# Quantum-Chemistry-Group-BNU/PyNQS

Hardware: AMD Instinct MI355X
Metric: local energies/sec (whole node) (higher is better)
Workload: dtype f64

## Files before the change

### pynqs_amd/csrc/kernels_reduce_rowout.hip

```cpp
#include "reduce_list.h"

namespace pynqs {

template <int LEN, typename T>
#ifndef PYNQS_ROWOUT_WAVES
#define PYNQS_ROWOUT_WAVES 6
#endif
__global__ __launch_bounds__(kBlock) __attribute__((amdgpu_waves_per_eu(PYNQS_ROWOUT_WAVES, 8)))
void reduce_onepass_list_rowout_kernel(const uint64_t *__restrict__ bra, SDParams p, PlanLayout pl, uint32_t nchunks, uint32_t chunk_len, uint32_t max_tiles,
                                       const T *__restrict__ plan, T eps, uint32_t nsample, uint64_t seed, uint32_t P, OnepassOut<T> o) {
  reduce_onepass_list_body<LEN, T, true, false, false, false, true>(bra, p, pl, nchunks, chunk_len, max_tiles, plan, eps, nsample, seed, P, o);
}

template <int LEN, typename T, bool GTILE>
__global__ __launch_bounds__(kBlock) void reduce_onepass_list_flush_row32_kernel(const uint64_t *__restrict__ bra, SDParams p, PlanLayout pl, uint32_t nchunks,
                                                                                uint32_t chunk_len, uint32_t max_tiles, const T *__restrict__ plan, T eps,
                                                                                uint32_t nsample, uint64_t seed, uint32_t P, OnepassOut<T> o) {
  reduce_onepass_list_body<LEN, T, true, false, true, GTILE, false, true>(bra, p, pl, nchunks, chunk_len, max_tiles, plan, eps, nsample, seed, P, o);
}

int launch_reduce_flush_row32(const uint64_t *bra, int64_t nbatch, const SDParams &p, const PlanLayout &pl, uint32_t chunk_len, uint32_t max_tiles,
                              const void *plan, int dtype, double eps_eff, int eps_sample, uint64_t seed, uint32_t P, size_t lds,
                              const pynqs_reduce_io *io, uint32_t fixed, bool gtile, hipStream_t st) {
  if (!io->row_f32) return set_error(PYNQS_EINVAL, "io->row_f32 missing");
  const int len = (p.sorb - 1) / 64 + 1;
#define PYNQS_R32_LAUNCH(TT)                                                                                                             \
  do {                                                                                                                                   \
    auto kfn = gtile ? reduce_onepass_list_flush_row32_kernel<LEN, TT, true> : reduce_onepass_list_flush_row32_kernel<LEN, TT, false>;   \
    if (lds > 64 * 1024 && hipFuncSetAttribute(reinterpret_cast<const void *>(kfn), hipFuncAttributeMaxDynamicSharedMemorySize, (int)lds) != hipSuccess) \
      return check_launch("hipFuncSetAttribute");                                                                                       \
    hipLaunchKernelGGL(kfn, dim3((uint32_t)nbatch), dim3(kBlock), lds, st, bra, p, pl, 1u, chunk_len, max_tiles, (const TT *)plan, (TT)eps_eff, \
                       (uint32_t)eps_sample, seed, P, make_out<TT>(io, len, fixed, gtile ? max_tiles : 0u));                            \
  } while (0)
  DISPATCH_LEN(len, {
    if (dtype == PYNQS_F64) PYNQS_R32_LAUNCH(double); else PYNQS_R32_LAUNCH(float);
  });
#undef PYNQS_R32_LAUNCH
  return check_launch("reduce_onepass (semi-stochastic, flushing, float32 row copy)");
}

bool reduce_draw_supported(const SDParams &p, int eps_sample) {
  return eps_sample > 0 && (uint32_t)eps_sample <= kDrawMaxDraws && p.nsd + 1 <= kDrawMaxCols;
}

int launch_reduce_rowout(const uint64_t *bra, int64_t nbatch, const SDParams &p, const PlanLayout &pl, uint32_t chunk_len, uint32_t max_tiles,
                         const void *plan, int dtype, double eps_eff, int eps_sample, uint64_t seed, uint32_t P, size_t lds,
                         const pynqs_reduce_io *io, uint32_t fixed, hipStream_t st) {
  if (!io->row_f32) return set_error(PYNQS_EINVAL, "io->row_f32 missing");
  const int len = (p.sorb - 1) / 64 + 1;
#define PYNQS_RO_LAUNCH(TT)                                                                                                              \
  do {                                                                                                                                   \
    auto kfn = reduce_onepass_list_rowout_kernel<LEN, TT>;                                                                               \
    if (lds > 64 * 1024 && hipFuncSetAttribute(reinterpret_cast<const void *>(kfn), hipFuncAttributeMaxDynamicSharedMemorySize, (int)lds) != hipSuccess) \
      return check_launch("hipFuncSetAttribute");                                                                                       \
    hipLaunchKernelGGL(kfn, dim3((uint32_t)nbatch), dim3(kBlock), lds, st, bra, p, pl, 1u, chunk_len, max_tiles, (const TT *)plan, (TT)eps_eff, \
                       (uint32_t)eps_sample, seed, P, make_out<TT>(io, len, fixed, 0u));                                                 \
  } while (0)
  DISPATCH_LEN(len, {
    if (dtype == PYNQS_F64) PYNQS_RO_LAUNCH(double); else PYNQS_RO_LAUNCH(float);
  });
#undef PYNQS_RO_LAUNCH
  return check_launch("reduce_onepass (semi-stochastic, sorted draws)");
}

}

#ifdef PYNQS_OP_STAMPS
extern "C" int pynqs_debug_stamps(unsigned long long *out) {
  return (int)hipMemcpyFromSymbol(out, HIP_SYMBOL(pynqs::g_stamps), sizeof(unsigned long long) * 8192 * 16);
}
#endif
```

### pynqs_amd/csrc/reduce_draw.h

```cpp
#pragma once
#include "reduce_common.h"

namespace pynqs {

constexpr int kDrawSeg = 16;
constexpr uint32_t kDrawMaxCols = 2u * kBlock * kDrawSeg, kDrawMaxDraws = 16383;
constexpr uint32_t kNoRec = 0xffffffffu;

__host__ __device__ inline size_t draw_lds_bytes(uint32_t nsample) {
  auto al = [](size_t b) { return (b + 15) & ~(size_t)15; };
  (void)nsample;
  return al((size_t)(2 * kBlock + 1) * 8) + (size_t)kBlock * 8;
}
__host__ __device__ inline size_t draw_row_stride(uint32_t ncomb) { return ((size_t)ncomb + kDrawSeg - 1) & ~(size_t)(kDrawSeg - 1); }

template <typename T, int K>
__device__ __forceinline__ void probe_k_oneword(const OnepassOut<T> &o, const uint64_t (&ket)[K][1], const bool (&act)[K], int32_t (&lk)[K],
                                                bool (&won)[K], int32_t (&rowhint)[K], uint32_t *full_flag) {
  uint32_t s[K];
  bool open[K];
  const bool full = *full_flag != 0u;
#pragma unroll
  for (int k = 0; k < K; ++k) {
    won[k] = false; rowhint[k] = -1;
    open[k] = act[k] && !full && !(o.debug & 1u);
    if (act[k]) lk[k] = -1;
    s[k] = (uint32_t)(hash_of<1>(ket[k]) >> 17) & o.dedup_mask;
  }
  for (uint32_t probes = 0;; ++probes) {
    unsigned long long cur[K];
    int32_t rw[K];
    if constexpr (K == 4) {
      typedef uint32_t u4 __attribute__((ext_vector_type(4)));
      u4 x0, x1, x2, x3;
      const uint64_t *a0 = o.dedup + (open[0] ? (size_t)s[0] * 2 : 0), *a1 = o.dedup + (open[1] ? (size_t)s[1] * 2 : 0),
                     *a2 = o.dedup + (open[2] ? (size_t)s[2] * 2 : 0), *a3 = o.dedup + (open[3] ? (size_t)s[3] * 2 : 0);
      asm volatile("global_load_dwordx4 %0, %4, off sc1\n\t"
                   "global_load_dwordx4 %1, %5, off sc1\n\t"
                   "global_load_dwordx4 %2, %6, off sc1\n\t"
                   "global_load_dwordx4 %3, %7, off sc1\n\t"
                   "s_waitcnt vmcnt(0)"
                   : "=&v"(x0), "=&v"(x1), "=&v"(x2), "=&v"(x3)
                   : "v"(a0), "v"(a1), "v"(a2), "v"(a3)
                   : "memory");
      cur[0] = ((unsigned long long)x0[1] << 32) | x0[0]; rw[0] = (int32_t)x0[2];
      cur[1] = ((unsigned long long)x1[1] << 32) | x1[0]; rw[1] = (int32_t)x1[2];
      cur[2] = ((unsigned long long)x2[1] << 32) | x2[0]; rw[2] = (int32_t)x2[2];
      cur[3] = ((unsigned long long)x3[1] << 32) | x3[0]; rw[3] = (int32_t)x3[2];
    } else {
#pragma unroll
      for (int k = 0; k < K; ++k) {
        cur[k] = 0ull; rw[k] = -1;
        if (open[k]) {
          unsigned long long *kp = reinterpret_cast<unsigned long long *>(o.dedup + (size_t)s[k] * 2);
          cur[k] = __hip_atomic_load(kp, __ATOMIC_RELAXED, __HIP_MEMORY_SCOPE_AGENT);
          rw[k] = __hip_atomic_load(reinterpret_cast<int32_t *>(kp + 1), __ATOMIC_RELAXED, __HIP_MEMORY_SCOPE_AGENT);
        }
      }
    }
#pragma unroll
    for (int k = 0; k < K; ++k) {
      if (open[k] && cur[k] == ~0ull && (o.debug & 2048u)) { open[k] = false; continue; }
      if (open[k] && cur[k] == ~0ull) {
        unsigned long long *kp = reinterpret_cast<unsigned long long *>(o.dedup + (size_t)s[k] * 2);
        cur[k] = atomicCAS(kp, ~0ull, (unsigned long long)ket[k][0]);
        if (cur[k] == ~0ull) { won[k] = true; lk[k] = (int32_t)s[k]; open[k] = false; }
        else rw[k] = -1;
      }
    }
    bool any = false;
#pragma unroll
    for (int k = 0; k < K; ++k) {
      if (open[k]) {
        if (cur[k] == ket[k][0]) { lk[k] = (int32_t)s[k]; rowhint[k] = rw[k]; open[k] = false; }
        else { s[k] = (s[k] + 1) & o.dedup_mask; any = true; }
      }
    }
    if (!any) break;
    if (probes + 1 >= kProbeLimit) {
      atomicOr(reinterpret_cast<unsigned int *>(o.counters + 1), 2u);
      *full_flag = 1u;
      break;
    }
  }
}

template <typename V>
__device__ __forceinline__ V draw_block_scan(V v, V *s_part, V *total) {
  const int lane = threadIdx.x & 63, wave = threadIdx.x >> 6;
  V incl = v;
#pragma unroll
  for (int d = 1; d < 64; d <<= 1) {
    const V ov = __shfl_up(incl, d);
    if (lane >= d) incl += ov;
  }
  __syncthreads();
  if (lane == 63) s_part[wave] = incl;
  __syncthreads();
  V before = V(0), tot = V(0);
#pragma unroll
  for (int w = 0; w < kBlock / 64; ++w) {
    if (w < wave) before += s_part[w];
    tot += s_part[w];
  }
  *total = tot;
  return before + incl;
}

template <int LEN, typename T>
__device__ __forceinline__ void rowout_draws(unsigned char *lds, uint32_t *rec, const uint32_t *kcol, uint32_t nkept, int64_t seg_base, const SDParams &p,
                                             const LdsLayout &L, const Walker<LEN> &wk, const float *__restrict__ w, uint32_t nsample, uint64_t seed,
                                             uint64_t walker, double Srow, const OnepassOut<T> &o, uint32_t *bw_cnt, int32_t *bw_base, uint32_t *s_full,
                                             double *s_part, uint32_t *s_parti) {
  constexpr int NT = kBlock, K = 4, SEG = kDrawSeg;
  typedef float f4 __attribute__((ext_vector_type(4)));
  const int tid = threadIdx.x;
  const uint32_t ncomb = p.nsd + 1;
  const uint32_t nseg = (ncomb + SEG - 1) / SEG, nbw = (ncomb + 31) / 32;
  const int64_t sbase = (int64_t)walker * nsample;
  auto al = [](size_t b) { return (b + 15) & ~(size_t)15; };
  double *pfx = reinterpret_cast<double *>(lds);
  uint32_t *bitmap = reinterpret_cast<uint32_t *>(lds + al((size_t)(2 * NT + 1) * 8));
  uint32_t *kpre = bitmap + NT;
  double ls[2];
#pragma unroll
  for (int h = 0; h < 2; ++h) {
    const uint32_t sgm = 2u * (uint32_t)tid + h;
    double a = 0.0;
    if (sgm < nseg) {
#pragma unroll
      for (int q4 = 0; q4 < SEG / 4; ++q4) {
        const f4 x = *reinterpret_cast<const f4 *>(w + (size_t)sgm * SEG + 4 * q4);
        a += (double)fabsf(x[0]); a += (double)fabsf(x[1]); a += (double)fabsf(x[2]); a += (double)fabsf(x[3]);
      }
    }
    ls[h] = a;
  }
  bitmap[tid] = 0u;
  for (uint32_t i = tid; i < nsample; i += NT) rec[i] = 0u;
  double total;
  const double incl = draw_block_scan<double>(ls[0] + ls[1], s_part, &total);
  pfx[2 * tid] = incl - (ls[0] + ls[1]);
  pfx[2 * tid + 1] = incl - ls[1];
  if (tid == NT - 1) pfx[2 * NT] = total;
  __syncthreads();
#ifdef PYNQS_OP_STAMPS
  if (threadIdx.x == 0 && walker < 8192) g_stamps[walker][7] = wall_clock64();
#endif
  const double scale = Srow / (double)nsample;
  const uint64_t key = op_mix64((o.seed_dev ? seed + *o.seed_dev : seed) ^ op_mix64(walker));
  const bool any_width = total > 0.0;
  if (o.debug & 64u) return;
  for (uint32_t k0 = 0; k0 < nsample; k0 += K * NT) {
    uint32_t dcol[K];
#pragma unroll 1
    for (int jj = 0; jj < K; ++jj) {
      const uint32_t k = k0 + (uint32_t)jj * NT + (uint32_t)tid;
      uint32_t found = kNoRec;
      if (k < nsample && any_width) {
        const uint64_t r = op_mix64(key ^ ((uint64_t)(k + 1u) * 0x9e3779b97f4a7c15ull));
        const double target = (double)(r >> 11) * 0x1.0p-53 * total;
        uint32_t lo = 0, hi = 2 * NT;
#pragma unroll
        for (int it = 0; it < 9; ++it) {
          const uint32_t mid = (lo + hi) >> 1;
          if (pfx[mid] <= target) lo = mid; else hi = mid;
        }
        if (lo >= nseg) lo = nseg - 1;
        const double res = target - pfx[lo];
        double acc = 0.0;
        int kf = -1, klast = -1;
        uint32_t neg = 0;
#pragma unroll
        for (int q4 = 0; q4 < SEG / 4; ++q4) {
          const f4 x = *reinterpret_cast<const f4 *>(w + (size_t)lo * SEG + 4 * q4);
#pragma unroll
          for (int e = 0; e < 4; ++e) {
            const double a = (double)fabsf(x[e]);
            acc += a;
            if (a > 0.0) {
              klast = 4 * q4 + e;
              if (kf < 0 && acc > res) kf = 4 * q4 + e;
            }
            neg |= (x[e] < 0.0f ? 1u : 0u) << (4 * q4 + e);
          }
        }
        if (kf < 0) kf = klast;
        if (kf >= 0) found = (lo * SEG + (uint32_t)kf) | (((neg >> kf) & 1u) << 15);
        else {
          for (uint32_t c = lo * SEG; c < ncomb && found == kNoRec; ++c)
            if (fabsf(w[c]) > 0.0f) found = c | ((w[c] < 0.0f ? 1u : 0u) << 15);
          for (int32_t c = (int32_t)(lo * SEG) - 1; c >= 0 && found == kNoRec; --c)
            if (fabsf(w[c]) > 0.0f) found = (uint32_t)c | ((w[c] < 0.0f ? 1u : 0u) << 15);
        }
        if (found != kNoRec) atomicOr(&bitmap[(found & 0x7fffu) >> 5], 1u << (found & 31u));
      }
      dcol[jj] = found;
    }
    __syncthreads();
    if (k0 + K * NT >= nsample) {
      uint32_t dummy;
      const uint32_t c = tid < (int)nbw ? (uint32_t)__popc(bitmap[tid]) : 0u;
      const uint32_t inc = draw_block_scan<uint32_t>(c, s_parti, &dummy);
      kpre[tid] = inc - c;
      __syncthreads();
    }
    if (nsample > K * NT) {
#pragma unroll
      for (int jj = 0; jj < K; ++jj) {
        const uint32_t k = k0 + (uint32_t)jj * NT + (uint32_t)tid;
        if (k < nsample) o.srec_link[sbase + k] = (int32_t)dcol[jj];
      }
    } else {
#pragma unroll
      for (int jj = 0; jj < K; ++jj) {
        const uint32_t f = dcol[jj];
        if (f != kNoRec) {
          const uint32_t c = f & 0x7fffu, wd = c >> 5;
          const uint32_t r = kpre[wd] + (uint32_t)__popc(bitmap[wd] & ((1u << (c & 31u)) - 1u));
          atomicAdd(&rec[r], 0x10000u);
          atomicOr(&rec[r], f);
        }
      }
    }
  }
  if (nsample > K * NT) {
    __syncthreads();
    for (uint32_t k = tid; k < nsample; k += NT) {
      const uint32_t f = (uint32_t)o.srec_link[sbase + k];
      if (f != kNoRec) {
        const uint32_t c = f & 0x7fffu, wd = c >> 5;
        const uint32_t r = kpre[wd] + (uint32_t)__popc(bitmap[wd] & ((1u << (c & 31u)) - 1u));
        atomicAdd(&rec[r], 0x10000u);
        atomicOr(&rec[r], f);
      }
    }
  }
  __syncthreads();
  const uint32_t nd = nbw ? kpre[nbw - 1] + (uint32_t)__popc(bitmap[nbw - 1]) : 0u;
#ifdef PYNQS_OP_STAMPS
  if (threadIdx.x == 0 && walker < 8192) g_stamps[walker][8] = wall_clock64();
#endif
  if (o.debug & 128u) return;
  constexpr int32_t kNoRecord = -0x7fffffff;
  for (uint32_t i = nd + tid; i < nsample; i += NT) __builtin_nontemporal_store((int32_t)-1, o.srec_col + sbase + i);
  const uint32_t nrec = nkept + nd;
  for (uint32_t i0 = 0; i0 < nrec; i0 += K * NT) {
    bool act[K], won[K];
    uint32_t slot[K];
    int32_t lk[K], rowhint[K];
    uint64_t ket[K][LEN];
    int64_t dst[K];
#pragma unroll
    for (int k = 0; k < K; ++k) {
      const uint32_t i = i0 + k * NT + tid;
      act[k] = false; won[k] = false; slot[k] = 0; lk[k] = kNoRecord; rowhint[k] = -1; dst[k] = 0;
#pragma unroll
      for (int ww = 0; ww < LEN; ++ww) ket[k][ww] = wk.w[ww];
      if (i >= nrec) continue;
      uint32_t col;
      if (i < nkept) {
        col = kcol[i];
        if (col == kNoRec) continue;
        dst[k] = seg_base + i;
      } else {
        const uint32_t e = rec[i - nkept];
        col = e & 0x7fffu;
        const int64_t at = sbase + (i - nkept);
        dst[k] = -1 - at;
        __builtin_nontemporal_store((int32_t)col, o.srec_col + at);
        const double val = scale * (double)(e >> 16);
        __builtin_nontemporal_store((T)(((e >> 15) & 1u) ? -val : val), o.srec_w + at);
      }
      act[k] = true;
      if (col) {
        const Excitation x = decode(col - 1, p, L);
        make_ket<LEN>(wk, x, ket[k]);
      }
      uint64_t *onv = dst[k] >= 0 ? o.rec_onv : o.srec_onv;
      if (onv) {
        const int64_t g = dst[k] >= 0 ? dst[k] : -1 - dst[k];
#pragma unroll
        for (int ww = 0; ww < LEN; ++ww) __builtin_nontemporal_store(ket[k][ww], onv + g * LEN + ww);
      }
    }
    bool fast = false;
    if constexpr (LEN == 1) fast = o.dedup != nullptr && o.lut == nullptr;
    if (fast) {
      if constexpr (LEN == 1) probe_k_oneword<T, K>(o, ket, act, lk, won, rowhint, s_full);
    } else {
#pragma unroll
      for (int k = 0; k < K; ++k)
        if (act[k]) lk[k] = probe_amplitude<LEN, T>(o, ket[k], won[k], s_full);
    }
#pragma unroll
    for (int k = 0; k < K; ++k) slot[k] = (uint32_t)lk[k];
    int32_t rows[K];
    allocate_batch_k<LEN, T, K>(o, p.sorb, won, slot, ket, bw_cnt, bw_base, rows);
#pragma unroll
    for (int k = 0; k < K; ++k) {
      if (!act[k]) continue;
      int32_t link;
      if (lk[k] >= 0 && rows[k] < 0 && rowhint[k] >= 0 && (uint32_t)rowhint[k] < o.ucap) link = rowhint[k] | kDirectLink;
      else if (o.debug & 4096u) link = lk[k];
      else link = final_link<LEN, T>(o, lk[k], rows[k]);
      __builtin_nontemporal_store(link, dst[k] >= 0 ? o.rec_link + dst[k] : o.srec_link + (-1 - dst[k]));
    }
  }
}

}
```

### pynqs_amd/csrc/reduce_list.h

```cpp
#pragma once
#include "reduce_common.h"

namespace pynqs {

#ifdef PYNQS_OP_STAMPS
__device__ unsigned long long g_stamps[8192][16];
#define PYNQS_STAMP(k) do { if (threadIdx.x == 0 && walker < 8192) g_stamps[walker][k] = wall_clock64(); } while (0)
#define PYNQS_STAMP_MARK() unsigned long long stamp_mark_ = wall_clock64()
#define PYNQS_STAMP_ADD(k) do { const unsigned long long now_ = wall_clock64(); if (threadIdx.x == 0 && walker < 8192) g_stamps[walker][k] += now_ - stamp_mark_; stamp_mark_ = now_; } while (0)
#define PYNQS_STAMP_ZERO(k) do { if (threadIdx.x == 0 && walker < 8192) g_stamps[walker][k] = 0; } while (0)
#else
#define PYNQS_STAMP(k) do { } while (0)
#define PYNQS_STAMP_MARK() do { } while (0)
#define PYNQS_STAMP_ADD(k) do { } while (0)
#define PYNQS_STAMP_ZERO(k) do { } while (0)
#endif

}
#include "reduce_draw.h"
namespace pynqs {

struct DrawLds {
  double *prefix;
  uint32_t *cs;
// ... 54 lines not shown
    if constexpr (ROWOUT || ROW32) {
      if ((reinterpret_cast<uintptr_t>(frow + col) & 7u) == 0) {
        typedef float f2 __attribute__((ext_vector_type(2)));
        __builtin_nontemporal_store(f2{fabs(h0) >= eps ? 0.0f : (float)h0, fabs(h1) >= eps ? 0.0f : (float)h1}, reinterpret_cast<f2 *>(frow + col));
        add_nocache(col, h0); add_nocache(col + 1, h1);
        return;
      }
    }
    add(col, h0); add(col + 1, h1);
  }
  __device__ __forceinline__ void add_nocache(uint32_t col, T h) {
    const T a = fabs(h);
    if (a >= eps) {
      const uint32_t k = atomicAdd(list_n, 1u);
      if (k < cap) { list_key[k] = FLUSH ? (((unsigned long long)col << 32) | k | tag) : (((unsigned long long)col << 32) | k); rec_w[k] = h; }
      if constexpr (ROWOUT) atomicOr(&kbm[col >> 5], 1u << (col & 31u));
    } else if constexpr (SAMPLED && !CACHED) {
      sub += (double)a;
    }
  }
  __device__ __forceinline__ void flush() {
    if constexpr (SAMPLED && !CACHED) {
      if (tile == 0xffffffffu) return;
      const double s = op_wave_sum(sub);
      if ((threadIdx.x & 63) == 0) tsum[tile] = s;
    }
  }
  __device__ __forceinline__ void tile_begin(uint32_t t) {
    flush(); tile = t; sub = 0.0;
    if constexpr (FLUSH) tag = t ? (1ull << 63) : 0ull;
  }
};

template <int LEN, typename T>
struct ListDrawSink {
  T eps;
  DrawLds S;
  const uint32_t *dinfo;
  double scale;
  uint64_t key;
  int64_t sbase;
  int32_t *__restrict__ srec_col;
  T *__restrict__ srec_w;
  uint32_t *pend;
  uint32_t tile;
  bool nodraw = false;
  uint32_t info_cur = 0;
  const uint32_t *tlist = nullptr;
  uint32_t ndrawn = 0;
  __device__ __forceinline__ uint32_t remap(uint32_t k) const { return tlist ? (k < ndrawn ? tlist[k] : 0xffffffffu) : k; }

  __device__ __forceinline__ void entry(uint32_t idx, uint32_t col, T h, double incl) const {
    S.prefix[idx] = incl;
    S.cs[idx] = col | (h < T(0) ? 0x80000000u : 0u);
  }
  __device__ __forceinline__ double width(T h) const {
    const T a = fabs(h);
    return a >= eps ? 0.0 : (double)a;
  }
  __device__ __forceinline__ void one(uint32_t col, T h, const uint64_t (&)[LEN]) const {
    const int lane = threadIdx.x & 63;
    uint64_t m = __ballot(1);
    const double w = width(h);
    while (m) {
      const int b = __ffsll((long long)m) - 1;
      m &= m - 1;
      if (lane == b) {
        const uint32_t idx = *S.ncols;
        const double incl = *S.run + w;
        entry(idx, col, h, incl);
        *S.ncols = idx + 1;
        *S.run = incl;
      }
      __builtin_amdgcn_wave_barrier();
    }
  }
  __device__ __forceinline__ void pair(uint32_t col, T h0, T h1, const uint64_t (&)[LEN], const uint64_t (&)[LEN]) const {
    const int lane = threadIdx.x & 63;
    const uint32_t nact = (uint32_t)__popcll(__ballot(1));
    const double w0 = width(h0), w1 = width(h1);
    const double incl = op_scan(w0 + w1, lane);
    const uint32_t base = *S.ncols;
    const double run = *S.run;
    entry(base + 2 * lane, col, h0, run + incl - w1);
    entry(base + 2 * lane + 1, col + 1, h1, run + incl);
    const double total = __shfl(incl, (int)nact - 1);
    __builtin_amdgcn_wave_barrier();
    if (lane == 0) { *S.ncols = base + 2 * nact; *S.run = run + total; }
    __builtin_amdgcn_wave_barrier();
  }
  __device__ __forceinline__ void two(uint32_t c0, T h0, const uint64_t (&)[LEN], uint32_t c1, T h1, const uint64_t (&)[LEN]) const {
    const int lane = threadIdx.x & 63;
    const double w0 = width(h0), w1 = width(h1);
    const double i0 = op_scan(w0, lane), t0 = __shfl(i0, 63);
    const double i1 = op_scan(w1, lane), t1 = __shfl(i1, 63);
    const uint32_t base = *S.ncols;
    const double run = *S.run;
    entry(base + lane, c0, h0, run + i0);
    entry(base + 64 + lane, c1, h1, run + t0 + i1);
    __builtin_amdgcn_wave_barrier();
    if (lane == 0) { *S.ncols = base + 128; *S.run = run + t0 + t1; }
    __builtin_amdgcn_wave_barrier();
  }
  __device__ __forceinline__ void flush() {
    if (tile == 0xffffffffu) return;
    const int lane = threadIdx.x & 63;
    const uint32_t info = info_cur;
    const uint32_t draws = info & 0xffffu;
    const uint32_t ncols = *S.ncols;
    const double total = *S.run;
    if (draws == 0 || ncols == 0 || !(total > 0.0) || nodraw) return;
    for (uint32_t k = lane; k < draws; k += 64) {
      const uint64_t r = op_mix64(key ^ op_mix64(((uint64_t)tile << 32) | k));
      const double target = (double)(r >> 11) * 0x1.0p-53 * total;
      uint32_t lo = 0, hi = ncols;
      while (lo < hi) {
        const uint32_t mid = (lo + hi) >> 1;
        if (S.prefix[mid] > target) hi = mid; else lo = mid + 1;
      }
      if (lo >= ncols) lo = ncols - 1;
      while (lo > 0 && !(S.prefix[lo] > S.prefix[lo - 1])) --lo;
      atomicAdd(&S.hits[lo], 1u);
    }
    __builtin_amdgcn_wave_barrier();
    uint32_t pos = info >> 16;
    for (uint32_t i0 = 0; i0 < ncols; i0 += 64) {
      const uint32_t idx = i0 + lane;
      const uint32_t hc = idx < ncols ? S.hits[idx] : 0u;
      const uint64_t m = __ballot(hc != 0u);
      if (hc) {
        const uint32_t e = S.cs[idx], col = e & 0x7fffffffu;
        const uint32_t at = pos + __popcll(m & ((1ull << lane) - 1ull));
        srec_col[sbase + at] = (int32_t)col;
        const double v = scale * (double)hc;
        srec_w[sbase + at] = (T)((e >> 31) ? -v : v);
        pend[at] = col;
      }
      pos += __popcll(m);
    }
  }
  __device__ __forceinline__ bool skip_tile(uint32_t) const { return (info_cur & 0xffffu) == 0u; }
  __device__ __forceinline__ void tile_begin(uint32_t t) {
    flush();
    tile = t;
    info_cur = dinfo[t];
    if ((info_cur & 0xffffu) == 0u) return;
    const int lane = threadIdx.x & 63;
    __builtin_amdgcn_wave_barrier();
    for (int i = lane; i < kOneTileCols; i += 64) S.hits[i] = 0u;
    if (lane == 0) { *S.ncols = 0u; *S.run = 0.0; }
    __builtin_amdgcn_wave_barrier();
  }
};

#ifndef PYNQS_LIST_Q_SAMPLED
#define PYNQS_LIST_Q_SAMPLED 256
#endif
#ifndef PYNQS_LIST_Q_DET
#define PYNQS_LIST_Q_DET 256
#endif
__host__ __device__ constexpr int list_quarter(bool sampled) { return sampled ? PYNQS_LIST_Q_SAMPLED : PYNQS_LIST_Q_DET; }
__host__ __device__ inline size_t list_scratch_offset(const SDParams &p) { return (lds_fixed_bytes(p) + 15) & ~(size_t)15; }
__host__ __device__ inline size_t list_base_lds(const SDParams &p, size_t esz, bool sampled, bool cached, bool rowout = false) {
  if (rowout) {
    const size_t scratch = esz * (size_t)(list_quarter(sampled) * (kBlock / 64)), draw = draw_lds_bytes(0);
    return (list_scratch_offset(p) + (scratch > draw ? scratch : draw) + 15) & ~(size_t)15;
  }
  const size_t scratch = esz * (size_t)(list_quarter(sampled) * (kBlock / 64)), draw = (kBlock / 64) * kCachedDrawLdsPerWave;
  if (cached) return (list_scratch_offset(p) + (scratch > draw ? scratch : draw) + 15) & ~(size_t)15;
  return (lds_fixed_bytes(p) + scratch + 15) & ~(size_t)15;
}


__host__ __device__ inline size_t row32_scratch_bytes(size_t esz) { return esz * (size_t)(list_quarter(true) * (kBlock / 64)); }
__host__ __device__ inline size_t row32_pend_bytes(uint32_t nsample, bool gtile) { return (((size_t)nsample * 4 * (gtile ? 2 : 1)) + 15) & ~(size_t)15; }
__host__ __device__ inline bool row32_fits(size_t esz, uint32_t P, uint32_t nsample, bool gtile) {
  const size_t in_scratch = row32_scratch_bytes(esz) / kCachedDrawLdsPerWave;
  const size_t rest = in_scratch >= (size_t)(kBlock / 64) ? 0 : (size_t)(kBlock / 64) - in_scratch;
  return row32_pend_bytes(nsample, gtile) + rest * kCachedDrawLdsPerWave <= (size_t)P * 8;
}
__host__ __device__ inline size_t row32_draw_area(size_t esz, uint32_t nsample, bool gtile, int wave, bool &in_list) {
  const size_t in_scratch = row32_scratch_bytes(esz) / kCachedDrawLdsPerWave;
  in_list = (size_t)wave >= in_scratch;
  return in_list ? row32_pend_bytes(nsample, gtile) + ((size_t)wave - in_scratch) * kCachedDrawLdsPerWave : (size_t)wave * kCachedDrawLdsPerWave;
}

__host__ __device__ inline size_t onepass_list_lds(const SDParams &p, size_t esz, uint32_t max_tiles, bool sampled, uint32_t P, uint32_t nsample,
                                                   bool cached, bool gtile = false, bool rowout = false, bool row32 = false) {
  size_t b = list_base_lds(p, esz, sampled, cached, rowout);
  if (sampled) {
    if (!gtile) {
      if (rowout) b += ((size_t)max_tiles * 8 + 15) & ~(size_t)15;
      else b += (size_t)max_tiles * 8 + (((size_t)max_tiles * 4 + 15) & ~(size_t)15);
    }
    if (!cached && !rowout && !row32) b += (kBlock / 64) * kDrawLdsPerWave;
  }
  if (rowout) {
    const size_t during = (((size_t)P * 8 + 15) & ~(size_t)15) + (size_t)kBlock * 4;
    const size_t after = (((size_t)P * 4 + 15) & ~(size_t)15) + (((size_t)nsample * 4 + 15) & ~(size_t)15);
    return b + (during > after ? during : after);
  }
  const size_t list = (size_t)P * 8, pend = (size_t)nsample * 4 * (gtile ? 2 : 1);
  return b + ((list > pend ? list : pend) + 15 & ~(size_t)15);
}

#ifndef PYNQS_U_LONG
#define PYNQS_U_LONG (3 * PYNQS_U)
#endif
__host__ __device__ constexpr int flush_tile_depth(int len, bool sampled, bool flush) { return (flush && !sampled && len >= 3) ? PYNQS_U_LONG : PYNQS_U; }
__host__ __device__ constexpr uint32_t flush_list_slots(int len, bool sampled, bool flush = true) {
  return flush_tile_depth(len, sampled, flush) > PYNQS_U ? 4096u : 2048u;
}
static_assert((kBlock / 64) * 128 * PYNQS_U_LONG + 64 < 4096 && (kBlock / 64) * 128 * PYNQS_U + 64 < 2048, "the pause threshold of the flushing form");

template <int LEN, typename T, bool SAMPLED, bool CACHED, bool FLUSH = false, bool GTILE = false, bool ROWOUT = false, bool ROW32 = false>
__device__ __forceinline__ void reduce_onepass_list_body(const uint64_t *__restrict__ bra, const SDParams &p, const PlanLayout &pl, uint32_t nchunks,
                                                         uint32_t chunk_len, uint32_t max_tiles, const T *__restrict__ plan, T eps,
                                                         uint32_t nsample, uint64_t seed, uint32_t P, OnepassOut<T> o) {
  extern __shared__ __attribute__((aligned(16))) unsigned char smem[];
  static_assert(!FLUSH || !CACHED, "the flushing form is for long rows: no row cache");
  __shared__ uint32_t next_tile, list_n, bw_cnt, s_done, s_full;
  __shared__ int32_t bw_base;
  __shared__ double s_part[kBlock / 64 + 1];
  __shared__ uint32_t s_parti[kBlock / 64 + 1];
  uint64_t walker;
  uint32_t chunk;
  map_workgroup(nchunks, false, walker, chunk);
  o.parent = (int32_t)walker;
  const uint64_t slot = walker * nchunks + chunk;
  const int tid = threadIdx.x, lane = tid & 63, wave = tid >> 6;
  const uint32_t cap = o.fixed + o.cap_d;
  const int64_t seg_base = (int64_t)slot * cap;
  if (tid == 0) { next_tile = 0; list_n = 0; bw_cnt = 0; s_done = 0; s_full = 0; }
  static_assert(!GTILE || (SAMPLED && !CACHED), "tile sums in global memory: the re-enumerating semi-stochastic form only");
  unsigned char *extra = smem + list_base_lds(p, sizeof(T), SAMPLED, CACHED, ROWOUT);
  unsigned char *tile_mem = GTILE ? o.tile_scratch + (size_t)walker * o.tile_stride : extra;
  double *tsum = reinterpret_cast<double *>(tile_mem);
  uint32_t *dinfo = reinterpret_cast<uint32_t *>(tile_mem + (SAMPLED ? (size_t)max_tiles * 8 : 0));
  unsigned char *after = (SAMPLED && !GTILE) ? (ROWOUT ? extra + (((size_t)max_tiles * 8 + 15) & ~(size_t)15)
                                                       : reinterpret_cast<unsigned char *>(dinfo) + (((size_t)max_tiles * 4 + 15) & ~(size_t)15)) : extra;
  unsigned char *draw0 = CACHED ? smem + list_scratch_offset(p) : after;
  static_assert(!ROWOUT || (SAMPLED && !CACHED && !FLUSH && !GTILE), "row to global memory as float32, the draws of reduce_draw.h");
  static_assert(!ROW32 || (SAMPLED && !CACHED && FLUSH && !ROWOUT), "float32 copy of a long row: the flushing semi-stochastic form");
  if (SAMPLED && !CACHED && !ROWOUT && !ROW32) after += (kBlock / 64) * kDrawLdsPerWave;
  unsigned long long *list_key = reinterpret_cast<unsigned long long *>(after);
  uint32_t *pend = reinterpret_cast<uint32_t *>(after);
  uint32_t *kbm = reinterpret_cast<uint32_t *>(after + (((size_t)P * 8 + 15) & ~(size_t)15));
  uint32_t *drec = reinterpret_cast<uint32_t *>(after + (((size_t)P * 4 + 15) & ~(size_t)15));
  if constexpr (SAMPLED) {
    for (uint32_t i = tid; i < max_tiles; i += kBlock) {
      tsum[i] = 0.0;
      if constexpr (!ROWOUT) dinfo[i] = 0u;
    }
    if constexpr (!ROWOUT) {
      for (uint32_t i = tid; i < nsample; i += kBlock) o.srec_col[(int64_t)walker * nsample + i] = -1;
    } else {
      for (size_t i = p.nsd + 1 + tid; i < draw_row_stride(p.nsd + 1); i += kBlock) o.row_f32[(size_t)walker * draw_row_stride(p.nsd + 1) + i] = 0.0f;
      kbm[tid] = 0u;
    }
  }
  Walker<LEN> wk;
  load_walker<LEN>(bra + walker * LEN, wk);
  const LdsLayout L = carve_lds(smem, p);
  PYNQS_STAMP(0);
  const int nocc = build_walker_tables<LEN>(wk, p, L);
  PYNQS_STAMP(1);
  uint32_t flushed = 0;
  uint32_t needed = 0;
  PYNQS_STAMP_ZERO(10); PYNQS_STAMP_ZERO(11); PYNQS_STAMP_ZERO(12); PYNQS_STAMP_ZERO(13);
  PYNQS_STAMP_MARK();
  for (;;) {
  const uint32_t room = FLUSH ? (cap > flushed ? min(cap - flushed, P) : 0u) : cap;
  {
    ListKeepSink<LEN, T, SAMPLED, CACHED, FLUSH, ROWOUT, ROW32> sink{eps, &list_n, list_key, o.rec_w + seg_base + flushed, room, tsum, 0xffffffffu, 0.0,
                                                                     CACHED ? o.row_cache + (size_t)walker * (p.nsd + 1) : nullptr};
    if constexpr (ROWOUT) { sink.frow = o.row_f32 + (size_t)walker * draw_row_stride(p.nsd + 1); sink.kbm = kbm; }
    if constexpr (ROW32) sink.frow = o.row_f32 + (size_t)walker * draw_row_stride(p.nsd + 1);
    constexpr int kUU = flush_tile_depth(LEN, SAMPLED, FLUSH);
    if constexpr (FLUSH) sink.pause_at = P - (kBlock / 64) * (kMaxKeptPerTile * kUU / PYNQS_U) - 64;
    const bool exhausted =
        visit_tiles<LEN, T, decltype(sink), true, list_quarter(SAMPLED), kUU>(p, pl, L, nocc, plan, wk, nchunks, chunk, chunk_len, 0u, &next_tile, sink);
    sink.flush();
    if (FLUSH && exhausted && lane == 0) s_done = 1u;
  }
  __syncthreads();
  if (o.debug & 32u) return;
  const bool last = !FLUSH || s_done != 0u;
  const uint32_t ntot = list_n;
  PYNQS_STAMP(2);
  if constexpr (FLUSH) PYNQS_STAMP_ADD(10);
  const uint32_t n = min(ntot, room);
  needed += ntot;
  if constexpr (!FLUSH) {
    if (tid == 0) {
      o.seg_count[slot] = (int32_t)(ntot > o.fixed ? ntot - o.fixed : 0u);
      if (ntot > cap) {
        atomicOr(reinterpret_cast<unsigned int *>(o.counters + 1), 1u);
        atomicMax(o.counters + 2, (int32_t)(ntot - o.fixed));
      }
    }
    for (uint32_t i = n + tid; i < o.fixed; i += kBlock) o.rec_col[seg_base + i] = -1;
  }
  if constexpr (ROWOUT) {
    uint32_t *kpre = reinterpret_cast<uint32_t *>(smem + list_scratch_offset(p));
    {
      uint32_t dummy;
      const uint32_t c = (uint32_t)__popc(kbm[tid]);
      const uint32_t inc = draw_block_scan<uint32_t>(c, s_parti, &dummy);
      kpre[tid] = inc - c;
    }
    __syncthreads();
    PYNQS_STAMP(3);
    constexpr int kMaxPer = 4;
    T mine_w[kMaxPer];
    uint32_t mine_c[kMaxPer], mine_r[kMaxPer];
#pragma unroll
    for (int r = 0; r < kMaxPer; ++r) {
      const uint32_t i = (uint32_t)r * kBlock + tid;
      mine_r[r] = 0xffffffffu; mine_c[r] = 0; mine_w[r] = T(0);
      if (i < n) {
        const unsigned long long e = list_key[i];
        mine_c[r] = (uint32_t)(e >> 32);
        mine_w[r] = o.rec_w[seg_base + (uint32_t)(e & 0xffffffffull)];
        mine_r[r] = kpre[mine_c[r] >> 5] + (uint32_t)__popc(kbm[mine_c[r] >> 5] & ((1u << (mine_c[r] & 31u)) - 1u));
      }
    }
    __syncthreads();
    uint32_t *kcol = reinterpret_cast<uint32_t *>(list_key);
    for (uint32_t i = tid; i < cap; i += kBlock) kcol[i] = 0xffffffffu;
    __syncthreads();
#pragma unroll
    for (int r = 0; r < kMaxPer; ++r) {
      if (mine_r[r] < cap) {
        __builtin_nontemporal_store(mine_w[r], o.rec_w + seg_base + mine_r[r]);
        __builtin_nontemporal_store((int32_t)mine_c[r], o.rec_col + seg_base + mine_r[r]);
        kcol[mine_r[r]] = mine_c[r];
      }
    }
    PYNQS_STAMP(4);
    PYNQS_STAMP(5);
    if (wave == 0) {
      double sl = 0.0;
      for (uint32_t i = lane; i < max_tiles; i += 64) sl += tsum[i];
      sl = op_wave_sum(sl);
      if (lane == 0) { s_part[kBlock / 64] = sl; if (o.row_sum) o.row_sum[walker] = sl; }
    }
    __syncthreads();
    const double Srow = s_part[kBlock / 64];
    __syncthreads();
    PYNQS_STAMP(6);
    rowout_draws<LEN, T>(smem + list_scratch_offset(p), drec, kcol, n, seg_base, p, L, wk, o.row_f32 + (size_t)walker * draw_row_stride(p.nsd + 1), nsample, seed,
                         walker, Srow, o, &bw_cnt, &bw_base, &s_full, s_part, s_parti);
    PYNQS_STAMP(9);
    return;
  }
  for (uint32_t i = n + tid; i < P; i += kBlock) list_key[i] = ~0ull;
  __syncthreads();
  PYNQS_STAMP(3);
  uint32_t Ps = 64;
  while (Ps < n) Ps <<= 1;
  for (uint32_t k = 2; k <= Ps; k <<= 1) {
    for (uint32_t j = k >> 1; j > 0; j >>= 1) {
      for (uint32_t i = tid; i < Ps; i += kBlock) {
        const uint32_t ixj = i ^ j;
        if (ixj > i) {
          const unsigned long long a = list_key[i], b = list_key[ixj];
          if ((a > b) == ((i & k) == 0)) {
            list_key[i] = b; list_key[ixj] = a;
          }
        }
      }
      __syncthreads();
    }
  }
  PYNQS_STAMP(4);
  if constexpr (FLUSH) PYNQS_STAMP_ADD(11);
  const int64_t out_base = seg_base + flushed;
  {
    constexpr int kMaxPer = (int)(flush_list_slots(LEN, SAMPLED, FLUSH) / kBlock);
    T mine_w[kMaxPer];
#pragma unroll
    for (int r = 0; r < kMaxPer; ++r) {
      const uint32_t i = (uint32_t)r * kBlock + tid;
      mine_w[r] = i < n ? o.rec_w[out_base + (uint32_t)(list_key[i] & 0xffffffffull)] : T(0);
    }
    __syncthreads();
#pragma unroll
    for (int r = 0; r < kMaxPer; ++r) {
      const uint32_t i = (uint32_t)r * kBlock + tid;
      if (i < n) o.rec_w[out_base + i] = mine_w[r];
    }
  }
  if constexpr (FLUSH) PYNQS_STAMP_ADD(12);
  for (uint32_t i0 = 0; i0 < n; i0 += kBlock) {
    const uint32_t i = i0 + tid;
    bool won = false;
    int32_t link = -1;
    uint64_t ket[LEN];
#pragma unroll
    for (int w = 0; w < LEN; ++w) ket[w] = wk.w[w];
    if (i < n) {
      const uint32_t col = (uint32_t)(list_key[i] >> 32) & (FLUSH ? 0x7fffffffu : 0xffffffffu);
      if (col) {
        const Excitation x = decode(col - 1, p, L);
        make_ket<LEN>(wk, x, ket);
      }
      const int64_t g = out_base + i;
      o.rec_col[g] = (int32_t)col;
      if (o.rec_onv) {
#pragma unroll
        for (int w = 0; w < LEN; ++w) o.rec_onv[g * LEN + w] = ket[w];
      }
      link = probe_amplitude<LEN, T>(o, ket, won, &s_full);
    }
    const int32_t mine = allocate_batch<LEN, T>(o, p.sorb, won, (uint32_t)link, ket, &bw_cnt, &bw_base);
    if (i < n) o.rec_link[out_base + i] = final_link<LEN, T>(o, link, mine);
  }
  flushed += n;
  if constexpr (FLUSH) PYNQS_STAMP_ADD(13);
  if (last) break;
  __syncthreads();
  if (tid == 0) list_n = 0;
  __syncthreads();
  }
  if constexpr (FLUSH) {
    if (tid == 0) {
      o.seg_count[slot] = (int32_t)(needed > o.fixed ? needed - o.fixed : 0u);
      if (needed > cap) {
        atomicOr(reinterpret_cast<unsigned int *>(o.counters + 1), 1u);
        atomicMax(o.counters + 2, (int32_t)(needed - o.fixed));
      }
    }
    for (uint32_t i = flushed + tid; i < o.fixed; i += kBlock) o.rec_col[seg_base + i] = -1;
  }
  PYNQS_STAMP(5);
  if constexpr (SAMPLED) {
    const uint32_t ncomb = p.nsd + 1;
    const T *__restrict__ hrow = CACHED ? o.row_cache + (size_t)walker * ncomb : nullptr;
    if constexpr (CACHED) {
      const uint32_t nct = (ncomb + kOneTileCols - 1) / kOneTileCols;
      for (uint32_t t = wave; t < nct; t += kBlock / 64) {
        double sl = 0.0;
#pragma unroll
        for (int j = 0; j < 4; ++j) {
          const uint32_t c = t * kOneTileCols + lane * 4 + j;
          const T a = c < ncomb ? fabs(hrow[c]) : T(0);
          sl += a >= eps ? 0.0 : (double)a;
        }
        sl = op_wave_sum(sl);
        if (lane == 0) tsum[t] = sl;
      }
      __syncthreads();
    }
    PYNQS_STAMP(6);
    const uint32_t per = (max_tiles + kBlock - 1) / kBlock;
    const uint32_t b0 = min((uint32_t)tid * per, max_tiles), b1 = min(b0 + per, max_tiles);
    double local = 0.0;
    for (uint32_t i = b0; i < b1; ++i) local += tsum[i];
    double incl = op_scan(local, lane);
    if (lane == 63) s_part[wave] = incl;
    for (uint32_t i = tid; i < nsample; i += kBlock) pend[i] = 0xffffffffu;
    __syncthreads();
    double before = 0.0, total = 0.0;
    for (int w = 0; w < kBlock / 64; ++w) {
      if (w < wave) before += s_part[w];
      total += s_part[w];
    }
    double run = before + incl - local;
    for (uint32_t i = b0; i < b1; ++i) { run += tsum[i]; tsum[i] = run; }
    __syncthreads();
    const double Srow = total;
    if (tid == 0 && o.row_sum) o.row_sum[walker] = Srow;
    const uint64_t key = op_mix64((o.seed_dev ? seed + *o.seed_dev : seed) ^ op_mix64(slot));
    if (Srow > 0.0) {
      for (uint32_t k = tid; k < nsample; k += kBlock) {
        const uint64_t r = op_mix64(key ^ op_mix64(0xffffffff00000000ull | k));
        const double target = (double)(r >> 11) * 0x1.0p-53 * Srow;
        uint32_t lo = 0, hi = max_tiles;
        while (lo < hi) {
          const uint32_t mid = (lo + hi) >> 1;
          if (tsum[mid] > target) hi = mid; else lo = mid + 1;
        }
        if (lo >= max_tiles) lo = max_tiles - 1;
        while (lo > 0 && !(tsum[lo] > tsum[lo - 1])) --lo;
        atomicAdd(&dinfo[lo], 1u);
      }
    }
    __syncthreads();
    uint32_t lsum = 0;
    for (uint32_t i = b0; i < b1; ++i) lsum += dinfo[i];
    uint32_t iscan = lsum;
#pragma unroll
    for (int d = 1; d < 64; d <<= 1) {
      const uint32_t ov = __shfl_up(iscan, d);
      if (lane >= d) iscan += ov;
    }
    if (lane == 63) s_parti[wave] = iscan;
    __syncthreads();
    uint32_t ibefore = 0;
    for (int w = 0; w < wave; ++w) ibefore += s_parti[w];
    uint32_t off = ibefore + iscan - lsum;
    for (uint32_t i = b0; i < b1; ++i) {
      const uint32_t c = dinfo[i];
      dinfo[i] = (off << 16) | c;
      off += c;
    }
    uint32_t *tlist = pend + nsample;
    uint32_t ndrawn = 0;
    if constexpr (GTILE) {
      uint32_t nd = 0;
      for (uint32_t i = b0; i < b1; ++i) nd += (dinfo[i] & 0xffffu) ? 1u : 0u;
      uint32_t dscan = nd;
#pragma unroll
      for (int d = 1; d < 64; d <<= 1) {
        const uint32_t ov = __shfl_up(dscan, d);
        if (lane >= d) dscan += ov;
      }
      __syncthreads();
      if (lane == 63) s_parti[wave] = dscan;
      __syncthreads();
      uint32_t dbefore = 0;
      for (int w = 0; w < kBlock / 64; ++w) {
        if (w < wave) dbefore += s_parti[w];
        ndrawn += s_parti[w];
      }
      uint32_t doff = dbefore + dscan - nd;
      for (uint32_t i = b0; i < b1; ++i)
        if (dinfo[i] & 0xffffu) tlist[doff++] = i;
    }
    if (tid == 0) next_tile = 0;
    __syncthreads();
    PYNQS_STAMP(7);
    unsigned char *mine = draw0 + (size_t)wave * (CACHED ? kCachedDrawLdsPerWave : kDrawLdsPerWave);
    if constexpr (ROW32) {
      bool in_list;
      const size_t off = row32_draw_area(sizeof(T), nsample, GTILE, wave, in_list);
      mine = (in_list ? after : smem + list_scratch_offset(p)) + off;
    }
    DrawLds S;
    S.prefix = reinterpret_cast<double *>(mine);
    S.run = reinterpret_cast<volatile double *>(mine + (size_t)kOneTileCols * 8);
    S.cs = reinterpret_cast<uint32_t *>(mine + (size_t)kOneTileCols * 8 + 8);
    S.hits = S.cs + kOneTileCols;
    S.ncols = reinterpret_cast<volatile uint32_t *>(S.hits + kOneTileCols);
    if constexpr (CACHED) {
      const uint32_t nct = (ncomb + kOneTileCols - 1) / kOneTileCols;
      const double scale = Srow / (double)nsample;
      const int64_t sbase = (int64_t)walker * nsample;
      for (;;) {
        uint32_t t = 0;
        if (lane == 0) t = atomicAdd(&next_tile, 1u);
        t = __builtin_amdgcn_readfirstlane(t);
        if (t >= nct) break;
        const uint32_t info = dinfo[t], draws = info & 0xffffu;
        if (draws == 0 || (o.debug & 64u)) continue;
        const uint32_t c0 = t * kOneTileCols + lane * 4;
        double w4[4];
        uint32_t neg = 0;
#pragma unroll
        for (int j = 0; j < 4; ++j) {
          const T h = c0 + j < ncomb ? hrow[c0 + j] : T(0);
          const T a = fabs(h);
          w4[j] = a >= eps ? 0.0 : (double)a;
          neg |= (h < T(0) ? 1u : 0u) << j;
        }
        const double ls = (w4[0] + w4[1]) + (w4[2] + w4[3]);
        const double incl = op_scan(ls, lane);
        const double total = __shfl(incl, 63);
        double run = incl - ls;
        __builtin_amdgcn_wave_barrier();
        uint32_t *hits2 = reinterpret_cast<uint32_t *>(mine + (size_t)kOneTileCols * 8);
#pragma unroll
        for (int j = 0; j < 4; ++j) {
          run += w4[j];
          S.prefix[lane * 4 + j] = run;
        }
        hits2[lane * 2] = 0u; hits2[lane * 2 + 1] = 0u;
        __builtin_amdgcn_wave_barrier();
        const uint32_t ncols = min((uint32_t)kOneTileCols, ncomb - t * kOneTileCols);
        if (!(total > 0.0)) continue;
        for (uint32_t k = lane; k < draws; k += 64) {
          const uint64_t r = op_mix64(key ^ op_mix64(((uint64_t)t << 32) | k));
          const double target = (double)(r >> 11) * 0x1.0p-53 * total;
          uint32_t lo = 0, hi = ncols;
          if (o.debug & 128u) { lo = (uint32_t)(r % ncols); hi = lo; }
          while (lo < hi) {
            const uint32_t mid = (lo + hi) >> 1;
            if (S.prefix[mid] > target) hi = mid; else lo = mid + 1;
          }
          if (lo >= ncols) lo = ncols - 1;
          while (lo > 0 && !(S.prefix[lo] > S.prefix[lo - 1])) --lo;
          atomicAdd(&hits2[lo >> 1], 1u << (16u * (lo & 1u)));
        }
        __builtin_amdgcn_wave_barrier();
        if (o.debug & 256u) continue;
        const uint32_t h01 = hits2[lane * 2], h23 = hits2[lane * 2 + 1];
        const uint32_t hc[4] = {h01 & 0xffffu, h01 >> 16, h23 & 0xffffu, h23 >> 16};
        const uint32_t mine = (hc[0] ? 1u : 0u) + (hc[1] ? 1u : 0u) + (hc[2] ? 1u : 0u) + (hc[3] ? 1u : 0u);
        uint32_t before = mine;
#pragma unroll
        for (int d = 1; d < 64; d <<= 1) {
          const uint32_t ov = __shfl_up(before, d);
          if (lane >= d) before += ov;
        }
        uint32_t at = (info >> 16) + before - mine;
#pragma unroll
        for (int j = 0; j < 4; ++j) {
          if (hc[j]) {
            const uint32_t col = c0 + j;
            o.srec_col[sbase + at] = (int32_t)col;
            const double v = scale * (double)hc[j];
            o.srec_w[sbase + at] = (T)(((neg >> j) & 1u) ? -v : v);
            pend[at] = col;
            ++at;
          }
        }
        __builtin_amdgcn_wave_barrier();
      }
    } else if constexpr (ROW32) {
      const TileGeom<LEN, true, PYNQS_U> geom(p, nchunks, chunk, chunk_len, 0u);
      const float *__restrict__ frow = o.row_f32 + (size_t)walker * draw_row_stride(p.nsd + 1);
      const double scale = Srow / (double)nsample;
      const int64_t sbase = (int64_t)walker * nsample;
      uint32_t *hits2 = reinterpret_cast<uint32_t *>(mine + (size_t)kOneTileCols * 8);
      for (;;) {
        uint32_t q = 0;
        if (lane == 0) q = atomicAdd(&next_tile, 1u);
        q = __builtin_amdgcn_readfirstlane(q);
        uint32_t t;
        if constexpr (GTILE) { if (q >= ndrawn) break; t = tlist[q]; }
        else { if (q >= geom.ntiles) break; t = q; }
        const uint32_t info = dinfo[t], draws = info & 0xffffu;
        if (draws == 0 || (o.debug & 64u)) continue;
        uint32_t c0 = 0, ncols = 0;
        if (t) geom.columns(t, c0, ncols);
        float x4[4];
        uint32_t cl[4];
#pragma unroll
        for (int j = 0; j < 4; ++j) {
          const uint32_t e = (uint32_t)lane * 4 + j;
          cl[j] = t ? (e < ncols ? c0 + e : 0xffffffffu) : geom.odd_column((int)e < 7 ? (int)e : 7);
          x4[j] = cl[j] != 0xffffffffu ? frow[cl[j]] : 0.0f;
        }
        const double w4[4] = {(double)fabsf(x4[0]), (double)fabsf(x4[1]), (double)fabsf(x4[2]), (double)fabsf(x4[3])};
        const double ls = (w4[0] + w4[1]) + (w4[2] + w4[3]);
        const double incl = op_scan(ls, lane);
        const double total = __shfl(incl, 63);
        double run = incl - ls;
        __builtin_amdgcn_wave_barrier();
#pragma unroll
        for (int j = 0; j < 4; ++j) {
          run += w4[j];
          S.prefix[lane * 4 + j] = run;
        }
        hits2[lane * 2] = 0u; hits2[lane * 2 + 1] = 0u;
// ... 90 lines not shown
```

Before: 9.620 million.

## Prefetch row segments early and software-pipeline draw location loads in pairs

The per-walker float32 row segments are now loaded into registers near the start of the rowout path, before the keep-list scan and row-sum reduction, so global-load latency overlaps that work. The draw loop is restructured to locate two draws at once and issue the next pair's segment loads while the current pair is walked, hiding gather latency. An optional, default-off stagger of first-round workgroups (env or macro controlled, with a cached occupancy query) is also added. The register prefetch raises register pressure, which may lower occupancy under the waves-per-eu hint.

```diff
diff --git a/pynqs_amd/csrc/kernels_reduce_rowout.hip b/pynqs_amd/csrc/kernels_reduce_rowout.hip
--- a/pynqs_amd/csrc/kernels_reduce_rowout.hip
+++ b/pynqs_amd/csrc/kernels_reduce_rowout.hip
@@ -1,6 +1,20 @@
 #include "reduce_list.h"
 
+#include <mutex>
+#include <vector>
+
 namespace pynqs {
+
+constexpr double kStaggerMaxUs = 1000.0;
+#ifndef PYNQS_ROWOUT_STAGGER_US
+#define PYNQS_ROWOUT_STAGGER_US 0.0
+#endif
+__device__ __forceinline__ void stagger_first_round(uint32_t ticks, uint32_t first_round) {
+  if (ticks == 0u || blockIdx.x >= first_round) return;
+  const uint32_t wait = (uint32_t)(((uint64_t)((blockIdx.x * 2654435761u) >> 8) * ticks) >> 24);
+  const unsigned long long t0 = wall_clock64();
+  for (uint32_t turn = 0, turns = wait / 8u + 1u; turn < turns && wall_clock64() - t0 < wait; ++turn) __builtin_amdgcn_s_sleep(8);
+}
 
 template <int LEN, typename T>
 #ifndef PYNQS_ROWOUT_WAVES
@@ -8,7 +22,9 @@
 #endif
 __global__ __launch_bounds__(kBlock) __attribute__((amdgpu_waves_per_eu(PYNQS_ROWOUT_WAVES, 8)))
 void reduce_onepass_list_rowout_kernel(const uint64_t *__restrict__ bra, SDParams p, PlanLayout pl, uint32_t nchunks, uint32_t chunk_len, uint32_t max_tiles,
-                                       const T *__restrict__ plan, T eps, uint32_t nsample, uint64_t seed, uint32_t P, OnepassOut<T> o) {
+                                       const T *__restrict__ plan, T eps, uint32_t nsample, uint64_t seed, uint32_t P, OnepassOut<T> o,
+                                       uint32_t stagger_ticks, uint32_t first_round) {
+  stagger_first_round(stagger_ticks, first_round);
   reduce_onepass_list_body<LEN, T, true, false, false, false, true>(bra, p, pl, nchunks, chunk_len, max_tiles, plan, eps, nsample, seed, P, o);
 }
 
@@ -43,18 +59,45 @@
   return eps_sample > 0 && (uint32_t)eps_sample <= kDrawMaxDraws && p.nsd + 1 <= kDrawMaxCols;
 }
 
+static uint32_t first_round_workgroups(const void *kfn, size_t lds) {
+  struct Entry { int dev; const void *kfn; size_t lds; uint32_t n; };
+  static std::mutex mu;
+  static std::vector<Entry> seen;
+  int dev = 0;
+  if (hipGetDevice(&dev) != hipSuccess) return 0u;
+  std::lock_guard<std::mutex> lock(mu);
+  for (const Entry &e : seen)
+    if (e.dev == dev && e.kfn == kfn && e.lds == lds) return e.n;
+  int per_cu = 0, cus = 0;
+  uint32_t n = 0;
+  if (hipOccupancyMaxActiveBlocksPerMultiprocessor(&per_cu, kfn, kBlock, lds) == hipSuccess &&
+      hipDeviceGetAttribute(&cus, hipDeviceAttributeMultiprocessorCount, dev) == hipSuccess && per_cu > 0 && cus > 0)
+    n = (uint32_t)per_cu * (uint32_t)cus;
+  else (void)hipGetLastError();
+  seen.push_back({dev, kfn, lds, n});
+  return n;
+}
+
 int launch_reduce_rowout(const uint64_t *bra, int64_t nbatch, const SDParams &p, const PlanLayout &pl, uint32_t chunk_len, uint32_t max_tiles,
                          const void *plan, int dtype, double eps_eff, int eps_sample, uint64_t seed, uint32_t P, size_t lds,
                          const pynqs_reduce_io *io, uint32_t fixed, hipStream_t st) {
   if (!io->row_f32) return set_error(PYNQS_EINVAL, "io->row_f32 missing");
   const int len = (p.sorb - 1) / 64 + 1;
+  const char *env = getenv("PYNQS_OP_STAGGER_US");
+  double stagger_us = env ? atof(env) : PYNQS_ROWOUT_STAGGER_US;
+  stagger_us = stagger_us > 0.0 ? (stagger_us < kStaggerMaxUs ? stagger_us : kStaggerMaxUs) : 0.0;
+  uint32_t stagger_ticks = (uint32_t)(stagger_us * 100.0), first_round = 0;
 #define PYNQS_RO_LAUNCH(TT)                                                                                                              \
   do {                                                                                                                                   \
     auto kfn = reduce_onepass_list_rowout_kernel<LEN, TT>;                                                                               \
     if (lds > 64 * 1024 && hipFuncSetAttribute(reinterpret_cast<const void *>(kfn), hipFuncAttributeMaxDynamicSharedMemorySize, (int)lds) != hipSuccess) \
       return check_launch("hipFuncSetAttribute");                                                                                       \
+    if (stagger_ticks) {                                                                                                                 \
+      first_round = first_round_workgroups(reinterpret_cast<const void *>(kfn), lds);                                                    \
+      if (first_round == 0u || (uint64_t)nbatch <= first_round) stagger_ticks = 0u;                                                      \
+    }                                                                                                                                    \
     hipLaunchKernelGGL(kfn, dim3((uint32_t)nbatch), dim3(kBlock), lds, st, bra, p, pl, 1u, chunk_len, max_tiles, (const TT *)plan, (TT)eps_eff, \
-                       (uint32_t)eps_sample, seed, P, make_out<TT>(io, len, fixed, 0u));                                                 \
+                       (uint32_t)eps_sample, seed, P, make_out<TT>(io, len, fixed, 0u), stagger_ticks, first_round);                     \
   } while (0)
   DISPATCH_LEN(len, {
     if (dtype == PYNQS_F64) PYNQS_RO_LAUNCH(double); else PYNQS_RO_LAUNCH(float);
diff --git a/pynqs_amd/csrc/reduce_draw.h b/pynqs_amd/csrc/reduce_draw.h
--- a/pynqs_amd/csrc/reduce_draw.h
+++ b/pynqs_amd/csrc/reduce_draw.h
@@ -107,13 +107,28 @@
   return before + incl;
 }
 
+typedef float draw_f4 __attribute__((ext_vector_type(4)));
+struct DrawRowSegments {
+  draw_f4 x[2][kDrawSeg / 4];
+};
+__device__ __forceinline__ void rowout_load_segments(const float *__restrict__ w, uint32_t ncomb, DrawRowSegments &s) {
+  const uint32_t nseg = (ncomb + kDrawSeg - 1) / kDrawSeg;
+#pragma unroll
+  for (int h = 0; h < 2; ++h) {
+    const uint32_t sgm = 2u * (uint32_t)threadIdx.x + h;
+#pragma unroll
+    for (int q4 = 0; q4 < kDrawSeg / 4; ++q4)
+      s.x[h][q4] = sgm < nseg ? *reinterpret_cast<const draw_f4 *>(w + (size_t)sgm * kDrawSeg + 4 * q4) : draw_f4{0.0f, 0.0f, 0.0f, 0.0f};
+  }
+}
+
 template <int LEN, typename T>
 __device__ __forceinline__ void rowout_draws(unsigned char *lds, uint32_t *rec, const uint32_t *kcol, uint32_t nkept, int64_t seg_base, const SDParams &p,
-                                             const LdsLayout &L, const Walker<LEN> &wk, const float *__restrict__ w, uint32_t nsample, uint64_t seed,
-                                             uint64_t walker, double Srow, const OnepassOut<T> &o, uint32_t *bw_cnt, int32_t *bw_base, uint32_t *s_full,
-                                             double *s_part, uint32_t *s_parti) {
+                                             const LdsLayout &L, const Walker<LEN> &wk, const float *__restrict__ w, const DrawRowSegments &segs,
+                                             uint32_t nsample, uint64_t seed, uint64_t walker, double Srow, const OnepassOut<T> &o, uint32_t *bw_cnt,
+                                             int32_t *bw_base, uint32_t *s_full, double *s_part, uint32_t *s_parti) {
   constexpr int NT = kBlock, K = 4, SEG = kDrawSeg;
-  typedef float f4 __attribute__((ext_vector_type(4)));
+  typedef draw_f4 f4;
   const int tid = threadIdx.x;
   const uint32_t ncomb = p.nsd + 1;
   const uint32_t nseg = (ncomb + SEG - 1) / SEG, nbw = (ncomb + 31) / 32;
@@ -125,14 +140,11 @@
   double ls[2];
 #pragma unroll
   for (int h = 0; h < 2; ++h) {
-    const uint32_t sgm = 2u * (uint32_t)tid + h;
     double a = 0.0;
-    if (sgm < nseg) {
-#pragma unroll
-      for (int q4 = 0; q4 < SEG / 4; ++q4) {
-        const f4 x = *reinterpret_cast<const f4 *>(w + (size_t)sgm * SEG + 4 * q4);
-        a += (double)fabsf(x[0]); a += (double)fabsf(x[1]); a += (double)fabsf(x[2]); a += (double)fabsf(x[3]);
-      }
+#pragma unroll
+    for (int q4 = 0; q4 < SEG / 4; ++q4) {
+      const f4 x = segs.x[h][q4];
+      a += (double)fabsf(x[0]); a += (double)fabsf(x[1]); a += (double)fabsf(x[2]); a += (double)fabsf(x[3]);
     }
     ls[h] = a;
   }
@@ -153,39 +165,49 @@
   if (o.debug & 64u) return;
   for (uint32_t k0 = 0; k0 < nsample; k0 += K * NT) {
     uint32_t dcol[K];
-#pragma unroll 1
-    for (int jj = 0; jj < K; ++jj) {
-      const uint32_t k = k0 + (uint32_t)jj * NT + (uint32_t)tid;
+    static_assert(K % 2 == 0, "the draws are located in pairs");
+    struct Located {
+      f4 x[SEG / 4];
+      uint32_t lo;
+      double res;
+    };
+    auto locate = [&](uint32_t k, Located &d) {
+      const uint64_t r = op_mix64(key ^ ((uint64_t)(k + 1u) * 0x9e3779b97f4a7c15ull));
+      const double target = (double)(r >> 11) * 0x1.0p-53 * total;
+      uint32_t lo = 0, hi = 2 * NT;
+#pragma unroll
+      for (int it = 0; it < 9; ++it) {
+        const uint32_t mid = (lo + hi) >> 1;
+        if (pfx[mid] <= target) lo = mid; else hi = mid;
+      }
+      if (lo >= nseg) lo = nseg - 1;
+      d.res = target - pfx[lo];
+      d.lo = (k < nsample && any_width) ? lo : 0u;
+#pragma unroll
+      for (int q4 = 0; q4 < SEG / 4; ++q4) d.x[q4] = *reinterpret_cast<const f4 *>(w + (size_t)d.lo * SEG + 4 * q4);
+    };
+    auto walk = [&](uint32_t k, const Located &d) -> uint32_t {
+      double acc = 0.0;
+      int kf = -1, klast = -1;
+      uint32_t neg = 0;
+#pragma unroll
+      for (int q4 = 0; q4 < SEG / 4; ++q4) {
+        const f4 x = d.x[q4];
+#pragma unroll
+        for (int e = 0; e < 4; ++e) {
+          const double a = (double)fabsf(x[e]);
+          acc += a;
+          if (a > 0.0) {
+            klast = 4 * q4 + e;
+            if (kf < 0 && acc > d.res) kf = 4 * q4 + e;
+          }
+          neg |= (x[e] < 0.0f ? 1u : 0u) << (4 * q4 + e);
+        }
+      }
+      if (kf < 0) kf = klast;
       uint32_t found = kNoRec;
       if (k < nsample && any_width) {
-        const uint64_t r = op_mix64(key ^ ((uint64_t)(k + 1u) * 0x9e3779b97f4a7c15ull));
-        const double target = (double)(r >> 11) * 0x1.0p-53 * total;
-        uint32_t lo = 0, hi = 2 * NT;
-#pragma unroll
-        for (int it = 0; it < 9; ++it) {
-          const uint32_t mid = (lo + hi) >> 1;
-          if (pfx[mid] <= target) lo = mid; else hi = mid;
-        }
-        if (lo >= nseg) lo = nseg - 1;
-        const double res = target - pfx[lo];
-        double acc = 0.0;
-        int kf = -1, klast = -1;
-        uint32_t neg = 0;
-#pragma unroll
-        for (int q4 = 0; q4 < SEG / 4; ++q4) {
-          const f4 x = *reinterpret_cast<const f4 *>(w + (size_t)lo * SEG + 4 * q4);
-#pragma unroll
-          for (int e = 0; e < 4; ++e) {
-            const double a = (double)fabsf(x[e]);
-            acc += a;
-            if (a > 0.0) {
-              klast = 4 * q4 + e;
-              if (kf < 0 && acc > res) kf = 4 * q4 + e;
-            }
-            neg |= (x[e] < 0.0f ? 1u : 0u) << (4 * q4 + e);
-          }
-        }
-        if (kf < 0) kf = klast;
+        const uint32_t lo = d.lo;
         if (kf >= 0) found = (lo * SEG + (uint32_t)kf) | (((neg >> kf) & 1u) << 15);
         else {
           for (uint32_t c = lo * SEG; c < ncomb && found == kNoRec; ++c)
@@ -195,7 +217,19 @@
         }
         if (found != kNoRec) atomicOr(&bitmap[(found & 0x7fffu) >> 5], 1u << (found & 31u));
       }
-      dcol[jj] = found;
+      return found;
+    };
+    Located A, B;
+    locate(k0 + (uint32_t)tid, A);
+    locate(k0 + (uint32_t)NT + (uint32_t)tid, B);
+#pragma unroll
+    for (int jj = 0; jj < K; jj += 2) {
+      const uint32_t k = k0 + (uint32_t)jj * NT + (uint32_t)tid;
+      const uint32_t fa = walk(k, A);
+      if (jj + 2 < K) locate(k + 2u * NT, A);
+      const uint32_t fb = walk(k + (uint32_t)NT, B);
+      if (jj + 2 < K) locate(k + 3u * NT, B);
+      dcol[jj] = fa; dcol[jj + 1] = fb;
     }
     __syncthreads();
     if (k0 + K * NT >= nsample) {
diff --git a/pynqs_amd/csrc/reduce_list.h b/pynqs_amd/csrc/reduce_list.h
--- a/pynqs_amd/csrc/reduce_list.h
+++ b/pynqs_amd/csrc/reduce_list.h
@@ -380,6 +380,9 @@
     for (uint32_t i = n + tid; i < o.fixed; i += kBlock) o.rec_col[seg_base + i] = -1;
   }
   if constexpr (ROWOUT) {
+    const float *__restrict__ frow = o.row_f32 + (size_t)walker * draw_row_stride(p.nsd + 1);
+    DrawRowSegments segs;
+    rowout_load_segments(frow, p.nsd + 1, segs);
     uint32_t *kpre = reinterpret_cast<uint32_t *>(smem + list_scratch_offset(p));
     {
       uint32_t dummy;
@@ -427,8 +430,8 @@
     const double Srow = s_part[kBlock / 64];
     __syncthreads();
     PYNQS_STAMP(6);
-    rowout_draws<LEN, T>(smem + list_scratch_offset(p), drec, kcol, n, seg_base, p, L, wk, o.row_f32 + (size_t)walker * draw_row_stride(p.nsd + 1), nsample, seed,
-                         walker, Srow, o, &bw_cnt, &bw_base, &s_full, s_part, s_parti);
+    rowout_draws<LEN, T>(smem + list_scratch_offset(p), drec, kcol, n, seg_base, p, L, wk, frow, segs, nsample, seed, walker, Srow, o, &bw_cnt, &bw_base,
+                         &s_full, s_part, s_parti);
     PYNQS_STAMP(9);
     return;
   }
```

New measurement: 9.486 million. -1.4%, worse.
